# moble/scri

Measured on AMD Instinct MI355X. Metric: timesteps/sec for full BMS transform, l_max=16, 1e5 steps; fp64, higher is better.
Workload: dtype f64

## Files before the change

scri_amd/csrc/kernels_gemm.hip:

```cpp
#include <cstdlib>
#include "kernels.h"

namespace bms {

typedef double v4d __attribute__((ext_vector_type(4)));

constexpr int G_BM = 128, G_BN = 128, G_BK = 16;
constexpr int G_LDA = G_BK + 2;
constexpr int G_LDB = G_BN + 16;
constexpr int G_ASZ = G_BM * G_LDA;
constexpr int G_BSZ = G_BK * G_LDB;

__global__ __launch_bounds__(256, 2) void dgemm_mfma_kernel(const double* __restrict__ A, long long lda,
                                                            const double* __restrict__ B, long long ldb,
                                                            double* __restrict__ C, long long ldc, long long M, int N,
                                                            int K, int nbm, int nbn, int st_rows_log2,
                                                            const double* __restrict__ col_off,
                                                            const double* __restrict__ col_scale) {
  __shared__ __attribute__((aligned(16))) double lds[2 * G_ASZ + 2 * G_BSZ];
  double* As = lds;
  double* Bs = lds + 2 * G_ASZ;

  const int b = blockIdx.x;
  const int xcd = b & 7;
  const int q = b >> 3;
  const int st_cols_log2 = 6 - st_rows_log2;
  const int nsn = (nbn + (1 << st_cols_log2) - 1) >> st_cols_log2;
  const int S = (q >> 6) * 8 + xcd;
  const int r = q & 63;
  const int bm = ((S / nsn) << st_rows_log2) + (r >> st_cols_log2);
  const int bn = ((S % nsn) << st_cols_log2) + (r & ((1 << st_cols_log2) - 1));
  if (bm >= nbm || bn >= nbn) return;
  const long long m0 = (long long)bm * G_BM;
  const int n0 = bn * G_BN;

  const int tid = threadIdx.x;
  const int wave = tid >> 6, lane = tid & 63;
  const int wm = wave >> 1, wn = wave & 1;
  const int fi = lane & 15, fk = lane >> 4;

  v4d acc[4][4];
#pragma unroll
  for (int i = 0; i < 4; ++i)
#pragma unroll
    for (int j = 0; j < 4; ++j) acc[i][j] = v4d{0.0, 0.0, 0.0, 0.0};

  double2 ra0, ra1, ra2, ra3, rb0, rb1, rb2, rb3;
  const int nk = (K + G_BK - 1) / G_BK;
  const int a_row = tid >> 3, a_ch = tid & 7;
  const int b_row = tid >> 6, b_ch = tid & 63;
  const double* a_ptr = A + (m0 + a_row) * lda + 2 * a_ch;
  const double* b_ptr = B + (long long)b_row * ldb + n0 + 2 * b_ch;
  const bool a_ok0 = (m0 + a_row) < M, a_ok1 = (m0 + a_row + 32) < M, a_ok2 = (m0 + a_row + 64) < M,
             a_ok3 = (m0 + a_row + 96) < M;
  const double2 zero2 = {0.0, 0.0};

#define G_LOAD_GLOBAL(kt)                                                                              \
  {                                                                                                    \
    const int k0 = (kt)*G_BK;                                                                          \
    const bool kok = (k0 + 2 * a_ch) < K;                                                              \
    ra0 = (a_ok0 && kok) ? *reinterpret_cast<const double2*>(a_ptr + k0) : zero2;                      \
    ra1 = (a_ok1 && kok) ? *reinterpret_cast<const double2*>(a_ptr + 32 * lda + k0) : zero2;           \
    ra2 = (a_ok2 && kok) ? *reinterpret_cast<const double2*>(a_ptr + 64 * lda + k0) : zero2;           \
    ra3 = (a_ok3 && kok) ? *reinterpret_cast<const double2*>(a_ptr + 96 * lda + k0) : zero2;           \
    const double* bp = b_ptr + (long long)k0 * ldb;                                                    \
    rb0 = *reinterpret_cast<const double2*>(bp);                                                       \
    rb1 = *reinterpret_cast<const double2*>(bp + 4 * ldb);                                             \
    rb2 = *reinterpret_cast<const double2*>(bp + 8 * ldb);                                             \
    rb3 = *reinterpret_cast<const double2*>(bp + 12 * ldb);                                            \
  }
#define G_STORE_LDS(buf)                                                                               \
  {                                                                                                    \
    double* as_w = As + (buf)*G_ASZ + a_row * G_LDA + 2 * a_ch;                                        \
    *reinterpret_cast<double2*>(as_w) = ra0;                                                           \
    *reinterpret_cast<double2*>(as_w + 32 * G_LDA) = ra1;                                              \
    *reinterpret_cast<double2*>(as_w + 64 * G_LDA) = ra2;                                              \
    *reinterpret_cast<double2*>(as_w + 96 * G_LDA) = ra3;                                              \
    double* bs_w = Bs + (buf)*G_BSZ + b_row * G_LDB + 2 * b_ch;                                        \
    *reinterpret_cast<double2*>(bs_w) = rb0;                                                           \
    *reinterpret_cast<double2*>(bs_w + 4 * G_LDB) = rb1;                                               \
    *reinterpret_cast<double2*>(bs_w + 8 * G_LDB) = rb2;                                               \
    *reinterpret_cast<double2*>(bs_w + 12 * G_LDB) = rb3;                                              \
  }

  G_LOAD_GLOBAL(0);
  G_STORE_LDS(0);
  __syncthreads();

  for (int kt = 0; kt < nk; ++kt) {
    const int buf = kt & 1;
    if (kt + 1 < nk) G_LOAD_GLOBAL(kt + 1);
    const double* as = As + buf * G_ASZ + (wm * 64 + fi) * G_LDA + fk;
    const double* bs = Bs + buf * G_BSZ + fk * G_LDB + wn * 64 + fi;
#pragma unroll
    for (int kk = 0; kk < G_BK / 4; ++kk) {
      double a[4], bb[4];
#pragma unroll
      for (int i = 0; i < 4; ++i) a[i] = as[i * 16 * G_LDA + kk * 4];
#pragma unroll
      for (int j = 0; j < 4; ++j) bb[j] = bs[kk * 4 * G_LDB + j * 16];
#pragma unroll
      for (int i = 0; i < 4; ++i)
#pragma unroll
        for (int j = 0; j < 4; ++j) acc[i][j] = __builtin_amdgcn_mfma_f64_16x16x4f64(a[i], bb[j], acc[i][j], 0, 0, 0);
    }
    if (kt + 1 < nk) G_STORE_LDS(buf ^ 1);
    __syncthreads();
  }

#pragma unroll
  for (int j = 0; j < 4; ++j) {
    const int col = n0 + wn * 64 + j * 16 + fi;
    if (col >= N) continue;
    const double off = col_off ? col_off[col] : 0.0;
    const double sc = col_scale ? col_scale[col] : 1.0;
#pragma unroll
    for (int i = 0; i < 4; ++i) {
#pragma unroll
      for (int r = 0; r < 4; ++r) {
        const long long row = m0 + wm * 64 + i * 16 + fk + 4 * r;
        if (row < M) C[row * ldc + col] = (acc[i][j][r] - off) * sc;
      }
    }
  }
}

#undef G_LOAD_GLOBAL
#undef G_STORE_LDS

constexpr int Z_BM = 64, Z_BN = 64, Z_KC = 8;
constexpr int Z_PA = 10;
constexpr int Z_PB = 64;
constexpr int Z_ASZ = Z_BM * Z_PA;
constexpr int Z_BSZ = Z_KC * Z_PB;

template <bool FOUR>
__global__ __launch_bounds__(256, FOUR ? 2 : 3) void zgemm3m_mfma_kernel(const double* __restrict__ A, long long lda,
                                                              const double* __restrict__ B, long long ldb,
                                                              double* __restrict__ C, long long ldc, long long M, int N,
                                                              int K, int nbm, int nbn, int st_rows_log2,
                                                              const double* __restrict__ col_off,
                                                              const double* __restrict__ col_scale) {
  __shared__ __attribute__((aligned(16))) double2 lds[2 * Z_ASZ + 2 * Z_BSZ];
  double2* As = lds;
  double2* Bs = lds + 2 * Z_ASZ;

  const int b = blockIdx.x;
  const int xcd = b & 7;
  const int q = b >> 3;
  const int st_cols_log2 = 6 - st_rows_log2;
  const int nsn = (nbn + (1 << st_cols_log2) - 1) >> st_cols_log2;
  const int S = (q >> 6) * 8 + xcd;
  const int r = q & 63;
  const int bm = ((S / nsn) << st_rows_log2) + (r >> st_cols_log2);
  const int bn = ((S % nsn) << st_cols_log2) + (r & ((1 << st_cols_log2) - 1));
  if (bm >= nbm || bn >= nbn) return;
  const long long m0 = (long long)bm * Z_BM;
  const int n0 = bn * Z_BN;

  const int tid = threadIdx.x;
  const int wave = tid >> 6, lane = tid & 63;
  const int wm = wave >> 1, wn = wave & 1;
  const int fi = lane & 15, fk = lane >> 4;

  v4d p1[2][2], p2[2][2], p3[2][2], p4[FOUR ? 2 : 1][FOUR ? 2 : 1];
#pragma unroll
  for (int i = 0; i < 2; ++i)
#pragma unroll
    for (int j = 0; j < 2; ++j) p1[i][j] = p2[i][j] = p3[i][j] = v4d{0.0, 0.0, 0.0, 0.0};
  if constexpr (FOUR) {
#pragma unroll
    for (int i = 0; i < 2; ++i)
#pragma unroll
      for (int j = 0; j < 2; ++j) p4[i][j] = v4d{0.0, 0.0, 0.0, 0.0};
  }

  const int a_row = tid >> 3, a_k = tid & 7;
  const int b_row = tid >> 6, b_col = tid & 63;
  const double* a_ptr = A + (m0 + a_row) * lda + 2 * a_k;
  const double* b_ptr = B + (long long)b_row * ldb + 2 * (n0 + b_col);
  const bool a_ok0 = (m0 + a_row) < M, a_ok1 = (m0 + a_row + 32) < M;
  const double2 zero2 = {0.0, 0.0};
  double2 ra0, ra1, rb0, rb1;
  const int nk = (K + Z_KC - 1) / Z_KC;

#define Z_LOAD_GLOBAL(kt)                                                                      \
  {                                                                                            \
    const int k0 = (kt)*Z_KC;                                                                  \
    const bool kok = (k0 + a_k) < K;                                                           \
    ra0 = (a_ok0 && kok) ? *reinterpret_cast<const double2*>(a_ptr + 2 * k0) : zero2;          \
    ra1 = (a_ok1 && kok) ? *reinterpret_cast<const double2*>(a_ptr + 32 * lda + 2 * k0) : zero2; \
    const double* bp = b_ptr + (long long)k0 * ldb;                                            \
    rb0 = *reinterpret_cast<const double2*>(bp);                                               \
    rb1 = *reinterpret_cast<const double2*>(bp + 4 * ldb);                                     \
  }
#define Z_STORE_LDS(buf)                                        \
  {                                                             \
    double2* as_w = As + (buf)*Z_ASZ + a_row * Z_PA + a_k;      \
    as_w[0] = ra0;                                              \
    as_w[32 * Z_PA] = ra1;                                      \
    double2* bs_w = Bs + (buf)*Z_BSZ + b_row * Z_PB + b_col;    \
    bs_w[0] = rb0;                                              \
    bs_w[4 * Z_PB] = rb1;                                       \
  }

  Z_LOAD_GLOBAL(0);
  Z_STORE_LDS(0);
  __syncthreads();

  const bool wave_has_columns = n0 + wn * 32 < N;
  for (int kt = 0; kt < nk; ++kt) {
    const int buf = kt & 1;
    if (kt + 1 < nk) Z_LOAD_GLOBAL(kt + 1);
    const double2* as = As + buf * Z_ASZ + (wm * 32 + fi) * Z_PA + fk;
    const double2* bs = Bs + buf * Z_BSZ + fk * Z_PB + wn * 32 + fi;
#pragma unroll
    for (int kk = 0; wave_has_columns && kk < Z_KC / 4; ++kk) {
      const double2 a0 = as[kk * 4], a1 = as[16 * Z_PA + kk * 4];
      const double2 b0 = bs[kk * 4 * Z_PB], b1 = bs[kk * 4 * Z_PB + 16];
      p1[0][0] = __builtin_amdgcn_mfma_f64_16x16x4f64(a0.x, b0.x, p1[0][0], 0, 0, 0);
      p1[0][1] = __builtin_amdgcn_mfma_f64_16x16x4f64(a0.x, b1.x, p1[0][1], 0, 0, 0);
      p1[1][0] = __builtin_amdgcn_mfma_f64_16x16x4f64(a1.x, b0.x, p1[1][0], 0, 0, 0);
      p1[1][1] = __builtin_amdgcn_mfma_f64_16x16x4f64(a1.x, b1.x, p1[1][1], 0, 0, 0);
      p2[0][0] = __builtin_amdgcn_mfma_f64_16x16x4f64(a0.y, b0.y, p2[0][0], 0, 0, 0);
      p2[0][1] = __builtin_amdgcn_mfma_f64_16x16x4f64(a0.y, b1.y, p2[0][1], 0, 0, 0);
      p2[1][0] = __builtin_amdgcn_mfma_f64_16x16x4f64(a1.y, b0.y, p2[1][0], 0, 0, 0);
      p2[1][1] = __builtin_amdgcn_mfma_f64_16x16x4f64(a1.y, b1.y, p2[1][1], 0, 0, 0);
      if constexpr (FOUR) {
        p3[0][0] = __builtin_amdgcn_mfma_f64_16x16x4f64(a0.x, b0.y, p3[0][0], 0, 0, 0);
        p3[0][1] = __builtin_amdgcn_mfma_f64_16x16x4f64(a0.x, b1.y, p3[0][1], 0, 0, 0);
        p3[1][0] = __builtin_amdgcn_mfma_f64_16x16x4f64(a1.x, b0.y, p3[1][0], 0, 0, 0);
        p3[1][1] = __builtin_amdgcn_mfma_f64_16x16x4f64(a1.x, b1.y, p3[1][1], 0, 0, 0);
        p4[0][0] = __builtin_amdgcn_mfma_f64_16x16x4f64(a0.y, b0.x, p4[0][0], 0, 0, 0);
        p4[0][1] = __builtin_amdgcn_mfma_f64_16x16x4f64(a0.y, b1.x, p4[0][1], 0, 0, 0);
        p4[1][0] = __builtin_amdgcn_mfma_f64_16x16x4f64(a1.y, b0.x, p4[1][0], 0, 0, 0);
        p4[1][1] = __builtin_amdgcn_mfma_f64_16x16x4f64(a1.y, b1.x, p4[1][1], 0, 0, 0);
      } else {
        const double sa0 = a0.x + a0.y, sa1 = a1.x + a1.y, sb0 = b0.x + b0.y, sb1 = b1.x + b1.y;
        p3[0][0] = __builtin_amdgcn_mfma_f64_16x16x4f64(sa0, sb0, p3[0][0], 0, 0, 0);
        p3[0][1] = __builtin_amdgcn_mfma_f64_16x16x4f64(sa0, sb1, p3[0][1], 0, 0, 0);
        p3[1][0] = __builtin_amdgcn_mfma_f64_16x16x4f64(sa1, sb0, p3[1][0], 0, 0, 0);
        p3[1][1] = __builtin_amdgcn_mfma_f64_16x16x4f64(sa1, sb1, p3[1][1], 0, 0, 0);
      }
    }
    if (kt + 1 < nk) Z_STORE_LDS(buf ^ 1);
    __syncthreads();
  }

#pragma unroll
  for (int j = 0; j < 2; ++j) {
    const int col = n0 + wn * 32 + j * 16 + fi;
    if (col >= N) continue;
    const double off_r = col_off ? col_off[2 * col] : 0.0, off_i = col_off ? col_off[2 * col + 1] : 0.0;
    const double sc_r = col_scale ? col_scale[2 * col] : 1.0, sc_i = col_scale ? col_scale[2 * col + 1] : 1.0;
#pragma unroll
    for (int i = 0; i < 2; ++i) {
#pragma unroll
      for (int rr = 0; rr < 4; ++rr) {
        const long long row = m0 + wm * 32 + i * 16 + fk + 4 * rr;
        if (row < M) {
          const double re = p1[i][j][rr] - p2[i][j][rr];
          double im;
          if constexpr (FOUR) im = p3[i][j][rr] + p4[i][j][rr];
          else im = (p3[i][j][rr] - p1[i][j][rr]) - p2[i][j][rr];
          double2 v;
          v.x = (re - off_r) * sc_r;
          v.y = (im - off_i) * sc_i;
          *reinterpret_cast<double2*>(C + row * ldc + 2LL * col) = v;
        }
      }
    }
  }
}

#undef Z_LOAD_GLOBAL
#undef Z_STORE_LDS

hipError_t launch_zgemm3m(hipStream_t stream, const double* A, long long lda, const double* B, long long ldb, double* C,
                          long long ldc, long long M, int N, int K, const double* col_off, const double* col_scale) {
  if (M <= 0 || N <= 0) return hipSuccess;
  const int nbm = (int)((M + Z_BM - 1) / Z_BM);
  const int nbn = (N + Z_BN - 1) / Z_BN;
  static const int st_env = BMS_PROBE_ENV("SCRI_AMD_ZGEMM_ST_ROWS_LOG2") ? atoi(BMS_PROBE_ENV("SCRI_AMD_ZGEMM_ST_ROWS_LOG2")) : -1;
  const int st_rows_log2 = (st_env >= 0 && st_env <= 6) ? st_env : (nbm >= 512 ? 6 : 5);
  const int sr = 1 << st_rows_log2, sc = 64 >> st_rows_log2;
  const long long n_super = (long long)((nbm + sr - 1) / sr) * ((nbn + sc - 1) / sc);
  const long long grid = ((n_super + 7) / 8) * 8 * 64;
  static const bool four = BMS_PROBE_ENV("SCRI_AMD_ZGEMM_4M") && atoi(BMS_PROBE_ENV("SCRI_AMD_ZGEMM_4M")) != 0;
  if (four)
    hipLaunchKernelGGL(zgemm3m_mfma_kernel<true>, dim3((unsigned)grid), dim3(256), 0, stream, A, lda, B, ldb, C, ldc, M, N,
                       K, nbm, nbn, st_rows_log2, col_off, col_scale);
  else
    hipLaunchKernelGGL(zgemm3m_mfma_kernel<false>, dim3((unsigned)grid), dim3(256), 0, stream, A, lda, B, ldb, C, ldc, M, N,
                       K, nbm, nbn, st_rows_log2, col_off, col_scale);
  return hipGetLastError();
}

hipError_t launch_dgemm(hipStream_t stream, const double* A, long long lda, const double* B, long long ldb, double* C,
                        long long ldc, long long M, int N, int K, const double* col_off, const double* col_scale) {
  if (M <= 0 || N <= 0) return hipSuccess;
  const int nbm = (int)((M + G_BM - 1) / G_BM);
  const int nbn = (N + G_BN - 1) / G_BN;
  static const int st_rows_log2 = BMS_PROBE_ENV("SCRI_AMD_GEMM_ST_ROWS_LOG2") ? atoi(BMS_PROBE_ENV("SCRI_AMD_GEMM_ST_ROWS_LOG2")) : 5;
  const int sr = 1 << st_rows_log2, sc = 64 >> st_rows_log2;
  const long long n_super = (long long)((nbm + sr - 1) / sr) * ((nbn + sc - 1) / sc);
  const long long grid = ((n_super + 7) / 8) * 8 * 64;
  hipLaunchKernelGGL(dgemm_mfma_kernel, dim3((unsigned)grid), dim3(256), 0, stream, A, lda, B, ldb, C, ldc, M, N, K, nbm,
                     nbn, st_rows_log2, col_off, col_scale);
  return hipGetLastError();
}

}
```

Baseline: 21.72 million.

## Use buffer-descriptor loads and narrow-tile wave remap in complex 3M GEMM

```diff
diff --git a/scri_amd/csrc/kernels_gemm.hip b/scri_amd/csrc/kernels_gemm.hip
--- a/scri_amd/csrc/kernels_gemm.hip
+++ b/scri_amd/csrc/kernels_gemm.hip
@@ -134,13 +134,16 @@
 constexpr int Z_ASZ = Z_BM * Z_PA;
 constexpr int Z_BSZ = Z_KC * Z_PB;
 
-template <bool FOUR>
+constexpr int Z_OOB = 0x7ffffff0;
+
+template <bool FOUR, bool DESC>
 __global__ __launch_bounds__(256, FOUR ? 2 : 3) void zgemm3m_mfma_kernel(const double* __restrict__ A, long long lda,
                                                               const double* __restrict__ B, long long ldb,
                                                               double* __restrict__ C, long long ldc, long long M, int N,
-                                                              int K, int nbm, int nbn, int st_rows_log2,
+                                                              int K, int nbm, int nbn, int st_rows_log2, unsigned nsn_magic,
                                                               const double* __restrict__ col_off,
                                                               const double* __restrict__ col_scale) {
+  static_assert(!(FOUR && DESC), "the 4-product form stays on the pointer loop");
   __shared__ __attribute__((aligned(16))) double2 lds[2 * Z_ASZ + 2 * Z_BSZ];
   double2* As = lds;
   double2* Bs = lds + 2 * Z_ASZ;
@@ -152,14 +155,16 @@
   const int nsn = (nbn + (1 << st_cols_log2) - 1) >> st_cols_log2;
   const int S = (q >> 6) * 8 + xcd;
   const int r = q & 63;
-  const int bm = ((S / nsn) << st_rows_log2) + (r >> st_cols_log2);
-  const int bn = ((S % nsn) << st_cols_log2) + (r & ((1 << st_cols_log2) - 1));
+  unsigned s_q = __umulhi((unsigned)S, nsn_magic), s_r = (unsigned)S - s_q * (unsigned)nsn;
+  if (s_r >= (unsigned)nsn) ++s_q, s_r -= (unsigned)nsn;
+  const int bm = (int)(s_q << st_rows_log2) + (r >> st_cols_log2);
+  const int bn = (int)(s_r << st_cols_log2) + (r & ((1 << st_cols_log2) - 1));
   if (bm >= nbm || bn >= nbn) return;
   const long long m0 = (long long)bm * Z_BM;
   const int n0 = bn * Z_BN;
 
   const int tid = threadIdx.x;
-  const int wave = tid >> 6, lane = tid & 63;
+  const int wave = __builtin_amdgcn_readfirstlane(tid >> 6), lane = tid & 63;
   const int wm = wave >> 1, wn = wave & 1;
   const int fi = lane & 15, fk = lane >> 4;
 
@@ -177,87 +182,149 @@
 
   const int a_row = tid >> 3, a_k = tid & 7;
   const int b_row = tid >> 6, b_col = tid & 63;
-  const double* a_ptr = A + (m0 + a_row) * lda + 2 * a_k;
-  const double* b_ptr = B + (long long)b_row * ldb + 2 * (n0 + b_col);
-  const bool a_ok0 = (m0 + a_row) < M, a_ok1 = (m0 + a_row + 32) < M;
-  const double2 zero2 = {0.0, 0.0};
   double2 ra0, ra1, rb0, rb1;
   const int nk = (K + Z_KC - 1) / Z_KC;
-
-#define Z_LOAD_GLOBAL(kt)                                                                      \
-  {                                                                                            \
-    const int k0 = (kt)*Z_KC;                                                                  \
-    const bool kok = (k0 + a_k) < K;                                                           \
-    ra0 = (a_ok0 && kok) ? *reinterpret_cast<const double2*>(a_ptr + 2 * k0) : zero2;          \
-    ra1 = (a_ok1 && kok) ? *reinterpret_cast<const double2*>(a_ptr + 32 * lda + 2 * k0) : zero2; \
-    const double* bp = b_ptr + (long long)k0 * ldb;                                            \
-    rb0 = *reinterpret_cast<const double2*>(bp);                                               \
-    rb1 = *reinterpret_cast<const double2*>(bp + 4 * ldb);                                     \
-  }
-#define Z_STORE_LDS(buf)                                        \
-  {                                                             \
-    double2* as_w = As + (buf)*Z_ASZ + a_row * Z_PA + a_k;      \
-    as_w[0] = ra0;                                              \
-    as_w[32 * Z_PA] = ra1;                                      \
-    double2* bs_w = Bs + (buf)*Z_BSZ + b_row * Z_PB + b_col;    \
-    bs_w[0] = rb0;                                              \
-    bs_w[4 * Z_PB] = rb1;                                       \
-  }
-
-  Z_LOAD_GLOBAL(0);
-  Z_STORE_LDS(0);
-  __syncthreads();
-
-  const bool wave_has_columns = n0 + wn * 32 < N;
-  for (int kt = 0; kt < nk; ++kt) {
-    const int buf = kt & 1;
-    if (kt + 1 < nk) Z_LOAD_GLOBAL(kt + 1);
-    const double2* as = As + buf * Z_ASZ + (wm * 32 + fi) * Z_PA + fk;
-    const double2* bs = Bs + buf * Z_BSZ + fk * Z_PB + wn * 32 + fi;
-#pragma unroll
-    for (int kk = 0; wave_has_columns && kk < Z_KC / 4; ++kk) {
-      const double2 a0 = as[kk * 4], a1 = as[16 * Z_PA + kk * 4];
-      const double2 b0 = bs[kk * 4 * Z_PB], b1 = bs[kk * 4 * Z_PB + 16];
-      p1[0][0] = __builtin_amdgcn_mfma_f64_16x16x4f64(a0.x, b0.x, p1[0][0], 0, 0, 0);
-      p1[0][1] = __builtin_amdgcn_mfma_f64_16x16x4f64(a0.x, b1.x, p1[0][1], 0, 0, 0);
-      p1[1][0] = __builtin_amdgcn_mfma_f64_16x16x4f64(a1.x, b0.x, p1[1][0], 0, 0, 0);
-      p1[1][1] = __builtin_amdgcn_mfma_f64_16x16x4f64(a1.x, b1.x, p1[1][1], 0, 0, 0);
-      p2[0][0] = __builtin_amdgcn_mfma_f64_16x16x4f64(a0.y, b0.y, p2[0][0], 0, 0, 0);
-      p2[0][1] = __builtin_amdgcn_mfma_f64_16x16x4f64(a0.y, b1.y, p2[0][1], 0, 0, 0);
-      p2[1][0] = __builtin_amdgcn_mfma_f64_16x16x4f64(a1.y, b0.y, p2[1][0], 0, 0, 0);
-      p2[1][1] = __builtin_amdgcn_mfma_f64_16x16x4f64(a1.y, b1.y, p2[1][1], 0, 0, 0);
-      if constexpr (FOUR) {
-        p3[0][0] = __builtin_amdgcn_mfma_f64_16x16x4f64(a0.x, b0.y, p3[0][0], 0, 0, 0);
-        p3[0][1] = __builtin_amdgcn_mfma_f64_16x16x4f64(a0.x, b1.y, p3[0][1], 0, 0, 0);
-        p3[1][0] = __builtin_amdgcn_mfma_f64_16x16x4f64(a1.x, b0.y, p3[1][0], 0, 0, 0);
-        p3[1][1] = __builtin_amdgcn_mfma_f64_16x16x4f64(a1.x, b1.y, p3[1][1], 0, 0, 0);
-        p4[0][0] = __builtin_amdgcn_mfma_f64_16x16x4f64(a0.y, b0.x, p4[0][0], 0, 0, 0);
-        p4[0][1] = __builtin_amdgcn_mfma_f64_16x16x4f64(a0.y, b1.x, p4[0][1], 0, 0, 0);
-        p4[1][0] = __builtin_amdgcn_mfma_f64_16x16x4f64(a1.y, b0.x, p4[1][0], 0, 0, 0);
-        p4[1][1] = __builtin_amdgcn_mfma_f64_16x16x4f64(a1.y, b1.x, p4[1][1], 0, 0, 0);
-      } else {
-        const double sa0 = a0.x + a0.y, sa1 = a1.x + a1.y, sb0 = b0.x + b0.y, sb1 = b1.x + b1.y;
+  double2* const as_w0 = As + a_row * Z_PA + a_k;
+  double2* const bs_w0 = Bs + b_row * Z_PB + b_col;
+  const auto store_lds = [&](int buf) __attribute__((always_inline)) {
+    double2* as_w = as_w0 + buf * Z_ASZ;
+    as_w[0] = ra0;
+    as_w[32 * Z_PA] = ra1;
+    double2* bs_w = bs_w0 + buf * Z_BSZ;
+    bs_w[0] = rb0;
+    bs_w[4 * Z_PB] = rb1;
+  };
+
+  const bool narrow = DESC && n0 + 32 >= N;
+  const int rbase = narrow ? wave * 16 : wm * 32, cbase = narrow ? 0 : wn * 32;
+  const bool wave_has_columns = n0 + cbase < N;
+  const double2* const as_r0 = As + (rbase + fi) * Z_PA + fk;
+  const double2* const bs_r0 = Bs + fk * Z_PB + cbase + fi;
+
+  if constexpr (DESC) {
+    const long long rows_valid = (M - m0) < Z_BM ? (M - m0) : Z_BM;
+    const double* a_base = A + m0 * lda;
+    const double* b_base = B + 2LL * n0;
+    const long long a_bytes = ((rows_valid - 1) * lda + 2LL * K) * 8;
+    const int b_bytes = (int)(((Z_KC - 1) * ldb + 2LL * Z_BN) * 8);
+    const int a_off0 = (int)(a_row * lda * 8) + 16 * a_k, a_off1 = a_off0 + (int)(32 * lda * 8);
+    const int b_off0 = (int)(b_row * ldb * 8) + 16 * b_col, b_off1 = b_off0 + (int)(4 * ldb * 8);
+    const bool k_tail = (nk - 1) * Z_KC + a_k >= K;
+    const int a_off0_last = k_tail ? Z_OOB : a_off0, a_off1_last = k_tail ? Z_OOB : a_off1;
+    const auto load_global = [&](int kt, bool last) __attribute__((always_inline)) {
+      const auto a_rs = __builtin_amdgcn_make_buffer_rsrc(const_cast<double*>(a_base + 2 * Z_KC * kt), 0, (int)(a_bytes - 16LL * Z_KC * kt), 0x00020000);
+      const auto b_rs = __builtin_amdgcn_make_buffer_rsrc(const_cast<double*>(b_base + (long long)kt * Z_KC * ldb), 0, b_bytes, 0x00020000);
+      ra0 = __builtin_bit_cast(double2, __builtin_amdgcn_raw_buffer_load_b128(a_rs, last ? a_off0_last : a_off0, 0, 0));
+      ra1 = __builtin_bit_cast(double2, __builtin_amdgcn_raw_buffer_load_b128(a_rs, last ? a_off1_last : a_off1, 0, 0));
+      rb0 = __builtin_bit_cast(double2, __builtin_amdgcn_raw_buffer_load_b128(b_rs, b_off0, 0, 0));
+      rb1 = __builtin_bit_cast(double2, __builtin_amdgcn_raw_buffer_load_b128(b_rs, b_off1, 0, 0));
+    };
+    load_global(0, nk == 1);
+    store_lds(0);
+    __syncthreads();
+    const auto turn = [&](int kt, int buf, bool more, bool last) __attribute__((always_inline)) {
+      if (more) load_global(kt + 1, last);
+      const double2* as = as_r0 + buf * Z_ASZ;
+      const double2* bs = bs_r0 + buf * Z_BSZ;
+#pragma unroll
+      for (int kk = 0; wave_has_columns && kk < Z_KC / 4; ++kk) {
+        const double2 a0 = as[kk * 4];
+        const double2 b0 = bs[kk * 4 * Z_PB], b1 = bs[kk * 4 * Z_PB + 16];
+        const double sa0 = a0.x + a0.y, sb0 = b0.x + b0.y, sb1 = b1.x + b1.y;
+        p1[0][0] = __builtin_amdgcn_mfma_f64_16x16x4f64(a0.x, b0.x, p1[0][0], 0, 0, 0);
+        p1[0][1] = __builtin_amdgcn_mfma_f64_16x16x4f64(a0.x, b1.x, p1[0][1], 0, 0, 0);
+        p2[0][0] = __builtin_amdgcn_mfma_f64_16x16x4f64(a0.y, b0.y, p2[0][0], 0, 0, 0);
+        p2[0][1] = __builtin_amdgcn_mfma_f64_16x16x4f64(a0.y, b1.y, p2[0][1], 0, 0, 0);
         p3[0][0] = __builtin_amdgcn_mfma_f64_16x16x4f64(sa0, sb0, p3[0][0], 0, 0, 0);
         p3[0][1] = __builtin_amdgcn_mfma_f64_16x16x4f64(sa0, sb1, p3[0][1], 0, 0, 0);
-        p3[1][0] = __builtin_amdgcn_mfma_f64_16x16x4f64(sa1, sb0, p3[1][0], 0, 0, 0);
-        p3[1][1] = __builtin_amdgcn_mfma_f64_16x16x4f64(sa1, sb1, p3[1][1], 0, 0, 0);
+        if (!narrow) {
+          const double2 a1 = as[16 * Z_PA + kk * 4];
+          const double sa1 = a1.x + a1.y;
+          p1[1][0] = __builtin_amdgcn_mfma_f64_16x16x4f64(a1.x, b0.x, p1[1][0], 0, 0, 0);
+          p1[1][1] = __builtin_amdgcn_mfma_f64_16x16x4f64(a1.x, b1.x, p1[1][1], 0, 0, 0);
+          p2[1][0] = __builtin_amdgcn_mfma_f64_16x16x4f64(a1.y, b0.y, p2[1][0], 0, 0, 0);
+          p2[1][1] = __builtin_amdgcn_mfma_f64_16x16x4f64(a1.y, b1.y, p2[1][1], 0, 0, 0);
+          p3[1][0] = __builtin_amdgcn_mfma_f64_16x16x4f64(sa1, sb0, p3[1][0], 0, 0, 0);
+          p3[1][1] = __builtin_amdgcn_mfma_f64_16x16x4f64(sa1, sb1, p3[1][1], 0, 0, 0);
+        }
       }
-    }
-    if (kt + 1 < nk) Z_STORE_LDS(buf ^ 1);
+      if (more) store_lds(buf ^ 1);
+      __syncthreads();
+    };
+    int kt = 0;
+    for (; kt + 3 < nk; kt += 2) {
+      turn(kt, 0, true, false);
+      turn(kt + 1, 1, true, false);
+    }
+    for (; kt < nk; ++kt) turn(kt, kt & 1, kt + 1 < nk, kt + 2 == nk);
+  } else {
+    const double* a_ptr = A + (m0 + a_row) * lda + 2 * a_k;
+    const double* b_ptr = B + (long long)b_row * ldb + 2 * (n0 + b_col);
+    const bool a_ok0 = (m0 + a_row) < M, a_ok1 = (m0 + a_row + 32) < M;
+    const double2 zero2 = {0.0, 0.0};
+    const auto load_global = [&](int kt) __attribute__((always_inline)) {
+      const int k0 = kt * Z_KC;
+      const bool kok = (k0 + a_k) < K;
+      ra0 = (a_ok0 && kok) ? *reinterpret_cast<const double2*>(a_ptr + 2 * k0) : zero2;
+      ra1 = (a_ok1 && kok) ? *reinterpret_cast<const double2*>(a_ptr + 32 * lda + 2 * k0) : zero2;
+      const double* bp = b_ptr + (long long)k0 * ldb;
+      rb0 = *reinterpret_cast<const double2*>(bp);
+      rb1 = *reinterpret_cast<const double2*>(bp + 4 * ldb);
+    };
+    load_global(0);
+    store_lds(0);
     __syncthreads();
+    for (int kt = 0; kt < nk; ++kt) {
+      const int buf = kt & 1;
+      if (kt + 1 < nk) load_global(kt + 1);
+      const double2* as = as_r0 + buf * Z_ASZ;
+      const double2* bs = bs_r0 + buf * Z_BSZ;
+#pragma unroll
+      for (int kk = 0; wave_has_columns && kk < Z_KC / 4; ++kk) {
+        const double2 a0 = as[kk * 4], a1 = as[16 * Z_PA + kk * 4];
+        const double2 b0 = bs[kk * 4 * Z_PB], b1 = bs[kk * 4 * Z_PB + 16];
+        p1[0][0] = __builtin_amdgcn_mfma_f64_16x16x4f64(a0.x, b0.x, p1[0][0], 0, 0, 0);
+        p1[0][1] = __builtin_amdgcn_mfma_f64_16x16x4f64(a0.x, b1.x, p1[0][1], 0, 0, 0);
+        p1[1][0] = __builtin_amdgcn_mfma_f64_16x16x4f64(a1.x, b0.x, p1[1][0], 0, 0, 0);
+        p1[1][1] = __builtin_amdgcn_mfma_f64_16x16x4f64(a1.x, b1.x, p1[1][1], 0, 0, 0);
+        p2[0][0] = __builtin_amdgcn_mfma_f64_16x16x4f64(a0.y, b0.y, p2[0][0], 0, 0, 0);
+        p2[0][1] = __builtin_amdgcn_mfma_f64_16x16x4f64(a0.y, b1.y, p2[0][1], 0, 0, 0);
+        p2[1][0] = __builtin_amdgcn_mfma_f64_16x16x4f64(a1.y, b0.y, p2[1][0], 0, 0, 0);
+        p2[1][1] = __builtin_amdgcn_mfma_f64_16x16x4f64(a1.y, b1.y, p2[1][1], 0, 0, 0);
+        if constexpr (FOUR) {
+          p3[0][0] = __builtin_amdgcn_mfma_f64_16x16x4f64(a0.x, b0.y, p3[0][0], 0, 0, 0);
+          p3[0][1] = __builtin_amdgcn_mfma_f64_16x16x4f64(a0.x, b1.y, p3[0][1], 0, 0, 0);
+          p3[1][0] = __builtin_amdgcn_mfma_f64_16x16x4f64(a1.x, b0.y, p3[1][0], 0, 0, 0);
+          p3[1][1] = __builtin_amdgcn_mfma_f64_16x16x4f64(a1.x, b1.y, p3[1][1], 0, 0, 0);
+          p4[0][0] = __builtin_amdgcn_mfma_f64_16x16x4f64(a0.y, b0.x, p4[0][0], 0, 0, 0);
+          p4[0][1] = __builtin_amdgcn_mfma_f64_16x16x4f64(a0.y, b1.x, p4[0][1], 0, 0, 0);
+          p4[1][0] = __builtin_amdgcn_mfma_f64_16x16x4f64(a1.y, b0.x, p4[1][0], 0, 0, 0);
+          p4[1][1] = __builtin_amdgcn_mfma_f64_16x16x4f64(a1.y, b1.x, p4[1][1], 0, 0, 0);
+        } else {
+          const double sa0 = a0.x + a0.y, sa1 = a1.x + a1.y, sb0 = b0.x + b0.y, sb1 = b1.x + b1.y;
+          p3[0][0] = __builtin_amdgcn_mfma_f64_16x16x4f64(sa0, sb0, p3[0][0], 0, 0, 0);
+          p3[0][1] = __builtin_amdgcn_mfma_f64_16x16x4f64(sa0, sb1, p3[0][1], 0, 0, 0);
+          p3[1][0] = __builtin_amdgcn_mfma_f64_16x16x4f64(sa1, sb0, p3[1][0], 0, 0, 0);
+          p3[1][1] = __builtin_amdgcn_mfma_f64_16x16x4f64(sa1, sb1, p3[1][1], 0, 0, 0);
+        }
+      }
+      if (kt + 1 < nk) store_lds(buf ^ 1);
+      __syncthreads();
+    }
   }
 
 #pragma unroll
   for (int j = 0; j < 2; ++j) {
-    const int col = n0 + wn * 32 + j * 16 + fi;
+    const int col = n0 + cbase + j * 16 + fi;
     if (col >= N) continue;
     const double off_r = col_off ? col_off[2 * col] : 0.0, off_i = col_off ? col_off[2 * col + 1] : 0.0;
     const double sc_r = col_scale ? col_scale[2 * col] : 1.0, sc_i = col_scale ? col_scale[2 * col + 1] : 1.0;
 #pragma unroll
     for (int i = 0; i < 2; ++i) {
+      if (i == 1 && narrow) continue;
 #pragma unroll
       for (int rr = 0; rr < 4; ++rr) {
-        const long long row = m0 + wm * 32 + i * 16 + fk + 4 * rr;
+        const long long row = m0 + rbase + i * 16 + fk + 4 * rr;
         if (row < M) {
           const double re = p1[i][j][rr] - p2[i][j][rr];
           double im;
@@ -273,9 +340,6 @@
   }
 }
 
-#undef Z_LOAD_GLOBAL
-#undef Z_STORE_LDS
-
 hipError_t launch_zgemm3m(hipStream_t stream, const double* A, long long lda, const double* B, long long ldb, double* C,
                           long long ldc, long long M, int N, int K, const double* col_off, const double* col_scale) {
   if (M <= 0 || N <= 0) return hipSuccess;
@@ -287,12 +351,18 @@
   const long long n_super = (long long)((nbm + sr - 1) / sr) * ((nbn + sc - 1) / sc);
   const long long grid = ((n_super + 7) / 8) * 8 * 64;
   static const bool four = BMS_PROBE_ENV("SCRI_AMD_ZGEMM_4M") && atoi(BMS_PROBE_ENV("SCRI_AMD_ZGEMM_4M")) != 0;
+  const unsigned nsn = (unsigned)((nbn + sc - 1) / sc);
+  const unsigned nsn_magic = nsn == 1 ? 0xffffffffu : (unsigned)(0x100000000ULL / nsn);
+  const bool desc = K > 0 && lda >= 2LL * K && lda * 8 * Z_BM < 0x7ffffff0LL && ldb * 8 * Z_KC + 16LL * Z_BN < 0x7ffffff0LL;
   if (four)
-    hipLaunchKernelGGL(zgemm3m_mfma_kernel<true>, dim3((unsigned)grid), dim3(256), 0, stream, A, lda, B, ldb, C, ldc, M, N,
-                       K, nbm, nbn, st_rows_log2, col_off, col_scale);
+    hipLaunchKernelGGL((zgemm3m_mfma_kernel<true, false>), dim3((unsigned)grid), dim3(256), 0, stream, A, lda, B, ldb, C, ldc, M,
+                       N, K, nbm, nbn, st_rows_log2, nsn_magic, col_off, col_scale);
+  else if (desc)
+    hipLaunchKernelGGL((zgemm3m_mfma_kernel<false, true>), dim3((unsigned)grid), dim3(256), 0, stream, A, lda, B, ldb, C, ldc, M,
+                       N, K, nbm, nbn, st_rows_log2, nsn_magic, col_off, col_scale);
   else
-    hipLaunchKernelGGL(zgemm3m_mfma_kernel<false>, dim3((unsigned)grid), dim3(256), 0, stream, A, lda, B, ldb, C, ldc, M, N,
-                       K, nbm, nbn, st_rows_log2, col_off, col_scale);
+    hipLaunchKernelGGL((zgemm3m_mfma_kernel<false, false>), dim3((unsigned)grid), dim3(256), 0, stream, A, lda, B, ldb, C, ldc, M,
+                       N, K, nbm, nbn, st_rows_log2, nsn_magic, col_off, col_scale);
   return hipGetLastError();
 }
 
```

After: 21.69 million. About the same (-0.2%).
